# maoqingyu1996/Boosting-Neural-Video-Representation-via-Online-Structural-Reparameteration

Hardware: AMD Instinct MI355X
Metric: training frames/sec, Bunny 720p ERB (higher is better)
Workload: dtype f16; 1 GPU; configs[1]: Bunny-shaped 132x3x720x1280 synthetic video, branch_type=ERB, fc_hw_dim 9_16_26, strides 5 2 2 2 2, stem 512_1, lower_width 96, Fusion6, Adam(0.5,0.999), b=1; one independent video per GPU; precision=fp16, hip_graph=False, launch_mode=stream, finite=True

## Files before the change

boosting-neural-video-representation-via-online-structural-reparameteration_amd/_lib.py:

```python
import ctypes
import os
from ctypes import POINTER, c_char_p, c_double, c_float, c_int, c_int32, c_int64, c_size_t, c_void_p

HERE = os.path.dirname(os.path.abspath(__file__))
ORN_MAX_LAYERS = 8
LOSS_TYPES = {'L2': 0, 'L1': 1, 'Fusion6': 2}


class OrnError(RuntimeError):
    pass


def lib_path() -> str:
    return os.environ.get('ORN_LIB_PATH') or os.path.join(HERE, 'liborn.so')


class LayerDesc(ctypes.Structure):
    _fields_ = [('C', c_int32), ('O', c_int32), ('s', c_int32), ('H', c_int32), ('W', c_int32),
                ('w3x3', c_int64), ('b3x3', c_int64), ('w3x1', c_int64), ('b3x1', c_int64),
                ('w1x3', c_int64), ('b1x3', c_int64), ('w1', c_int64), ('w2', c_int64), ('w3', c_int64)]


class EngineDesc(ctypes.Structure):
    _fields_ = [('n_layers', c_int32), ('erb', c_int32), ('embed_len', c_int32), ('stem_dim', c_int32),
# ... 54 lines not shown
    'orn_engine_train_steps': (c_int, [P, P, P, P, P, P, c_int32, c_int32, P]),
    'orn_engine_profile_step': (c_int, [P, P, P, P, P, P, c_int32, P, P]),
    'orn_engine_set_grad_mask': (c_int, [P, P]),
    'orn_engine_set_target_stats': (c_int, [P, P]),
    'orn_engine_fused_kernel': (c_int, [P, c_int, POINTER(c_void_p), POINTER(c_void_p)]),
    'orn_engine_scale_state': (c_int, [P, P]),
    'orn_engine_set_grad_scale': (c_int, [P, c_float, c_float]),
}
EXPORTS = tuple(_SIGS.keys())
_DEBUG_SIGS = {'orn_debug_set': (None, [c_int]), 'orn_debug_set_stamps': (None, [c_void_p]),
               'orn_debug_conv_fwd_bf16': (c_int, [P, P, P] + [c_int] * 5 + [P, P, c_int, P]),
               'orn_debug_conv_fwd_f16': (c_int, [P, P, P] + [c_int] * 5 + [P, P, c_int, P]),
               'orn_debug_conv_dgrad_bf16': (c_int, [P, P] + [c_int] * 4 + [P, P, c_int, P, c_int, P]),
               'orn_debug_conv_dgrad_f16': (c_int, [P, P] + [c_int] * 4 + [P, P, c_int, P, c_int, P]),
               'orn_debug_merge_h16_bwd': (c_int, [c_int, P, P, P, P, P]),
               'orn_debug_decode_out_ws_bytes': (c_size_t, []),
               'orn_debug_decode_out_f32': (c_int, [P, c_int, c_int, P, P, P, P, P, c_size_t, P])}

_lib = None


def lib():
    global _lib
    if _lib is None:
        path = lib_path()
        if not os.path.exists(path):
            raise OrnError(f'{path} is missing: build it with `python -c "import __graft_entry__ as g; g.build()"` '
                           '(hipcc --offload-arch=gfx950).  There is no CPU fallback.')
        L = ctypes.CDLL(path)
        for name, (res, args) in _SIGS.items():
# ... 37 lines not shown
```

boosting-neural-video-representation-via-online-structural-reparameteration_amd/csrc/orn_engine.hip:

```cpp
#include "orn_internal.h"
#include <new>
#include <cstdlib>
#include <cassert>

struct LayerBuf {
    float *T, *wf, *bf;
    float *w2t;
    float *dT, *dw1p;
    float *wd32;
    void *mh16;
    float *dw2t;
    float *z, *a;
    float *da;
    uint16_t *xpad;
    uint16_t *zb;
    uint16_t *dypad;
    uint16_t *wb, *wd;
    float *biasp;
    float *wslab;
};

struct orn_engine {
    orn_engine_desc d;
    float *params, *grads, *m, *v;
    const float *gmask;
    const float *tstats;
    float *ws;
    float *pre1, *h1, *pre2, *h2, *dh2;
    float *img, *dimg, *stats;
// ... 13 lines not shown
        int layer[ORN_MAX_LAYERS];
        void *tables;
        int tiles[4];
        void *mh_tables, *mh_host;
    } mset[3];
    int ff;
    float *dxn;
    size_t stem_ws;
    bool stage0;
    hipGraph_t graph, graph_u;
    hipGraphExec_t graph_exec, graph_exec_u;
    const void *g_frames, *g_embeds, *g_sched, *g_cursor, *g_stats;
    int g_slots;
    hipStream_t g_stream;
    hipStream_t side;
    hipEvent_t ev_fork, ev_adam, ev_wgrad, ev_join, ev_below;
    OrnStepCur *cur_side;
    OrnScaleState *sc_side;
    size_t side_lo;
    bool pipe_ok;
    bool side_below;
    bool fork_behind_dgrad;
    int last_smax;
    bool side_busy;
    bool prof;
    hipEvent_t prof_ev[4 * ORN_MAX_LAYERS + 4];
};

#define ORN_GRAPH_UNROLL 4
static_assert(ORN_SCALE_SLOTS >= ORN_GRAPH_UNROLL, "one scale-state entry per step of the unrolled graph");

static inline size_t al(size_t floats) { return orn_align(floats * 4) / 4; }

static hipEvent_t orn_engine::*const SIDE_EVENTS[] = {&orn_engine::ev_fork, &orn_engine::ev_adam, &orn_engine::ev_wgrad, &orn_engine::ev_join,
                                                      &orn_engine::ev_below};

static constexpr int ORN_LAST_SMAX = 24;

static void drop_graphs(orn_engine *e)
{
    if (e->graph_exec) { (void)hipGraphExecDestroy(e->graph_exec); e->graph_exec = nullptr; }
    if (e->graph) { (void)hipGraphDestroy(e->graph); e->graph = nullptr; }
    if (e->graph_exec_u) { (void)hipGraphExecDestroy(e->graph_exec_u); e->graph_exec_u = nullptr; }
    if (e->graph_u) { (void)hipGraphDestroy(e->graph_u); e->graph_u = nullptr; }
}

extern "C" size_t orn_conv3x3_ps_silu_bwd_ws_bytes(int B, int C, int O, int H, int W);
extern "C" size_t orn_erb_merge_bwd_ws_bytes(int C, int O);
extern "C" size_t orn_head_bwd_ws_bytes(int B, int C, int H, int W);
extern "C" size_t orn_loss_ws_bytes(int B, int Ch, int H, int W);
// ... 100 lines not shown
    if (s3 > scratch) scratch = s3;
    float *scr = take(scratch);
    const orn_layer_desc &ll = d->layer[d->n_layers - 1];
    float *head_ws = (ff < d->n_layers) ? take(orn_half_ops_bf16()->head_bwd_ws_floats(Cn))
                   : (ll.s == 2 ? take((size_t)(orn_head_bwd_fused_f32_blocks(ll.H, ll.W) + 1) * (3 * Cn + 3)) : nullptr);
    float *cur = take((sizeof(OrnStepCur) * ORN_GRAPH_UNROLL + 3) / 4 + 16);
    float *scs = take(sizeof(OrnScaleState) * ORN_SCALE_SLOTS / 4);
    float *mtab[3], *mhtab[3];
    for (int k = 0; k < 3; ++k) {
        mtab[k] = d->erb ? take(orn_merge_group_bytes() / 4) : nullptr;
        mhtab[k] = (d->erb && d->precision != 0) ? take(orn_merge_h16_table_bytes() / 4) : nullptr;
    }
    float *cur_side = take((sizeof(OrnStepCur) + 3) / 4 + 16);
    float *sc_side = take(sizeof(OrnScaleState) / 4 + 16);
    float *dec_ws = take(ORN_DECODE_WS_FLOATS);
    if (e) {
        e->pre1 = pre1; e->h1 = h1; e->pre2 = pre2; e->h2 = h2; e->dh2 = dh2;
        e->img = img; e->dimg = dimg; e->stats = stats; e->loss_ws = loss_ws; e->scratch = scr; e->head_ws = head_ws;
        e->cur = (OrnStepCur *)cur;
        e->sc = (OrnScaleState *)scs;
        for (int i = 0; i < d->n_layers; ++i) e->L[i] = L[i];
        e->Hout = H; e->Wout = W; e->Cn_last = Cn;
        e->ff = ff; e->dxn = dxn;
        e->stem_ws = al(orn_stem_bwd_ws_floats(1, d->stem_dim, Nout));
        const orn_layer_desc &l0 = d->layer[0];
        e->stage0 = d->precision != 0 && ff == 1 && d->n_layers > 1 && orn_stage0_supported(l0.C, l0.O, l0.H, l0.W, l0.s);
        for (int k = 0; k < 3; ++k) { e->mset[k].tables = mtab[k]; e->mset[k].mh_tables = mhtab[k]; }
        e->cur_side = (OrnStepCur *)cur_side;
        e->sc_side = (OrnScaleState *)sc_side;
        e->dec_ws = dec_ws;
// ... 20 lines not shown
        return ORN_E_WS;
    }
    ORN_TRY(orn_loss_init());
    orn_engine *e = new (std::nothrow) orn_engine();
    ORN_REQUIRE(e, "engine_create: out of host memory");
    e->d = *d;
    e->params = params; e->grads = grads; e->m = adam_m; e->v = adam_v;
    e->gmask = nullptr;
    e->tstats = nullptr;
    e->ws = (float *)ws;
    e->graph = nullptr; e->graph_exec = nullptr; e->graph_u = nullptr; e->graph_exec_u = nullptr;
    e->prof = false;
    for (int k = 0; k < 3; ++k) { e->mset[k].n = 0; e->mset[k].mh_host = nullptr; }
    e->side = nullptr;
    for (auto ev : SIDE_EVENTS) e->*ev = nullptr;
    e->pipe_ok = false; e->side_busy = false; e->side_lo = 0;
    for (int i = 0; i < 4 * ORN_MAX_LAYERS + 4; ++i) e->prof_ev[i] = nullptr;
    e->ops = (d->precision == 2) ? orn_half_ops_f16() : orn_half_ops_bf16();
    e->gs = (d->precision == 2) ? 1048576.0f : 1.0f;
    layout(d, e);
    {
        hipError_t rc = hipMemset(ws, 0, need);
        if (rc == hipSuccess) rc = hipDeviceSynchronize();
        if (rc != hipSuccess) { orn_set_error("engine_create: hipMemset failed: %s", hipGetErrorString(rc)); delete e; return (int)rc; }
        OrnScaleState s0[ORN_SCALE_SLOTS] = {};
        for (int r = 0; r < ORN_SCALE_SLOTS; ++r) { s0[r].gs = e->gs; s0[r].inv_gs = 1.0f / e->gs; s0[r].gs_max = e->gs; }
        rc = hipMemcpy(e->sc, s0, sizeof(s0), hipMemcpyHostToDevice);
        if (rc == hipSuccess) rc = hipMemcpy(e->sc_side, s0, sizeof(OrnScaleState), hipMemcpyHostToDevice);
        if (rc != hipSuccess) { orn_set_error("engine_create: scale state upload failed: %s", hipGetErrorString(rc)); delete e; return (int)rc; }
    }
    {
// ... 29 lines not shown
            e->L[i].wf = params + d->layer[i].w3x3;
            e->L[i].bf = params + d->layer[i].b3x3;
        }
    else {
        auto fill = [&](int i, OrnMergeLayer &m, bool half_in_S) {
            const orn_layer_desc &l = d->layer[i];
            m.C = l.C; m.O = l.O;
            m.w3x3 = params + l.w3x3; m.w3x1 = params + l.w3x1; m.w1x3 = params + l.w1x3;
            m.w1 = params + l.w1; m.w2 = params + l.w2; m.w3 = params + l.w3;
            m.T = e->L[i].T; m.wf = e->L[i].wf; m.w2t = e->L[i].w2t;
            m.b3x3 = params + l.b3x3; m.b1x3 = params + l.b1x3; m.b3x1 = params + l.b3x1; m.bf = e->L[i].bf;
            m.g = grads ? grads + l.w3x3 : nullptr;
            m.dT = e->L[i].dT; m.dw1p = e->L[i].dw1p;
            m.dw2 = grads ? grads + l.w2 : nullptr; m.dw3 = grads ? grads + l.w3 : nullptr;
            m.dw2t = e->L[i].dw2t;
            m.half_kind = 0; m.s2 = l.s * l.s; m.Cp = ORN_FAST_C; m.wb = m.wd = nullptr; m.biasp = nullptr;
            if (i >= e->ff && half_in_S) {
                m.half_kind = d->precision; m.wb = e->L[i].wb; m.wd = e->L[i].wd; m.biasp = e->L[i].biasp;
            }
        };
        const int nl = d->n_layers;
        for (int k = 0; k < (e->pipe_ok ? 3 : 1); ++k) {
            orn_engine::MergeSet &ms = e->mset[k];
            const int i0 = k == 2 ? nl - 1 : 0, i1 = k == 1 ? nl - 1 : nl;
            ms.n = 0;
            void *bufs[ORN_MAX_LAYERS];
            for (int i = i0; i < i1; ++i) {
                fill(i, ms.ml[ms.n], k == 2 || !e->stage0);
                bufs[ms.n] = e->L[i].mh16;
                ms.layer[ms.n++] = i;
// ... 122 lines not shown

static bool f32_head_on_z(const orn_engine *e)
{
    const orn_engine_desc &d = e->d;
    return e->ff >= d.n_layers && e->head_ws && d.layer[d.n_layers - 1].s == 2;
}

static int slab_cap(const orn_engine *e, int i) { return i == e->d.n_layers - 1 ? e->last_smax : 0; }

static OrnPrepLayer prep_layer(const orn_engine *e, int i)
{
    const orn_layer_desc &l = e->d.layer[i];
    return OrnPrepLayer{e->L[i].wf, e->L[i].bf, l.O, l.C, l.s, e->L[i].wb, e->L[i].wd, e->L[i].biasp, ORN_FAST_C};
}

static OrnWgradJob wgrad_job(const orn_engine *e, int i)
{
    const orn_layer_desc &l = e->d.layer[i];
    return OrnWgradJob{e->L[i].xpad, e->L[i].dypad, l.H, l.W, l.C, l.O, l.s, e->L[i].wslab, slab_cap(e, i)};
}

static OrnWgradReduce wgrad_reduce(const orn_engine *e, int i, OrnScaleState *sc)
{
    const orn_layer_desc &l = e->d.layer[i];
    return OrnWgradReduce{e->L[i].wslab, l.H, l.W, l.C, l.O, l.s, 1.0f / e->gs, e->grads + l.w3x3, e->grads + l.b3x3, sc, slab_cap(e, i)};
}

enum { MERGE_NONE = -1 };
static int forward(orn_engine *e, const float *embeds, const int *row_idx, bool keep_z, hipStream_t st, int set = 0, bool head = true)
{
    const bool merge = set != MERGE_NONE;
    const orn_engine_desc &d = e->d;
    const int Nout = d.fc_h * d.fc_w * d.fc_dim;
    float *P = e->params;
    const OrnLinearJob lin1 = {embeds, row_idx, (size_t)d.embed_len, P + d.stem_w0, P + d.stem_b0, 1, d.embed_len, d.stem_dim, e->pre1, e->h1};
    const OrnLinearJob lin2 = {e->h1, nullptr, 0, P + d.stem_w1, P + d.stem_b1, 1, d.stem_dim, Nout, e->pre2, e->h2};
    const float *x = e->h2;
    const int nl = d.n_layers, ff = e->ff;
    const void *pack_t = nullptr;
    int pack_t_blocks = 0;
// ... 28 lines not shown
                ORN_TRY(orn_launch_stage0_fwd(x, b.wf, b.bf, l.C, l.O, l.H, l.W, l.s, keep_z ? b.z : nullptr, e->L[1].xpad, ORN_FAST_C,
                                              d.precision, st, np, pl, pack_t, pack_t_blocks));
            }
            else
            {
                const bool z_only = keep_z && i == nl - 1 && f32_head_on_z(e);
                ORN_TRY(orn_launch_conv3x3_f32(x, b.wf, b.bf, 1, l.C, l.O, l.H, l.W, l.s, 1, keep_z ? b.z : nullptr, z_only ? nullptr : b.a, st, nullptr));
            }
            if (e->prof) (void)hipEventRecord(e->prof_ev[2 * i + 1], st);
            x = b.a;
        } else {
            if (i == ff && !e->stage0) ORN_TRY(e->ops->to_nhwc(x, l.C, ORN_FAST_C, l.H, l.W, b.xpad, st));
            if (e->prof) (void)hipEventRecord(e->prof_ev[2 * i], st);
            const bool last = (i + 1 == nl);
            if (e->side_busy && i + 3 == nl && e->side_below) ORN_HIP(hipStreamWaitEvent(st, e->ev_below, 0));
            if (e->side_busy && i + 2 == nl) ORN_HIP(hipStreamWaitEvent(st, e->ev_wgrad, 0));
            if (e->side_busy && last) { ORN_HIP(hipStreamWaitEvent(st, e->ev_join, 0)); e->side_busy = false; }
            ORN_TRY(e->ops->conv_fwd(b.xpad, b.wb, b.biasp, l.H, l.W, ORN_FAST_C, l.O, l.s, b.zb, last ? nullptr : e->L[i + 1].xpad, st, l.C));
            if (e->prof) (void)hipEventRecord(e->prof_ev[2 * i + 1], st);
        }
    }
    if (ff < nl) {
        if (head)
            ORN_TRY(e->ops->head_fwd(e->L[nl - 1].zb, P + d.head_w, P + d.head_b, e->Cn_last, (size_t)e->Hout * e->Wout, d.sigmoid, e->img, st));
    } else
    {
        const bool z_only = keep_z && f32_head_on_z(e);
        ORN_TRY(orn_launch_head_fwd(z_only ? e->L[nl - 1].z : x, P + d.head_w, P + d.head_b, 1, e->Cn_last, (size_t)e->Hout * e->Wout, d.sigmoid, e->img,
                                    st, z_only));
    }
    return 0;
}

// ... 93 lines not shown
    const orn_engine_desc &d = e->d;
    const int nl = d.n_layers;
    float *G = e->grads;
    hipStream_t sd = e->side;
    OrnScaleState *sc = e->sc_side;
    ORN_HIP(hipEventRecord(e->ev_fork, st));
    ORN_HIP(hipStreamWaitEvent(sd, e->ev_fork, 0));
    if (e->side_below) {
        const OrnWgradJob wb = wgrad_job(e, nl - 2);
        ORN_TRY(e->ops->wgrad_batch(1, &wb, sd, nullptr, nullptr, 1));
        ORN_HIP(hipEventRecord(e->ev_below, sd));
    }
    const OrnWgradJob wj = wgrad_job(e, nl - 1);
    const OrnHeadFinish hf = {e->head_ws, e->ops->head_bwd_blocks(e->Hout, e->Wout), e->Cn_last, 1.0f / e->gs, G + d.head_w, G + d.head_b, sc};
    ORN_TRY(e->ops->wgrad_batch(1, &wj, sd, &hf, nullptr, 1));
    ORN_HIP(hipEventRecord(e->ev_wgrad, sd));
    const OrnWgradReduce wr = wgrad_reduce(e, nl - 1, sc);
    ORN_TRY(e->ops->wgrad_reduce_all(1, &wr, sd, nullptr));
    if (d.erb) {
        const orn_engine::MergeSet &ms = e->mset[2];
        ORN_TRY(orn_launch_merge_h16_bwd(ms.mh_tables, ms.mh_host, sd, sc));
        const OrnMergeMisc mm = merge_misc(e, nl - 1);
        ORN_TRY(orn_launch_merge_bwd_tail_all(1, &mm, sd));
    }
    return 0;
}

static int side_branch_update(orn_engine *e, bool more)
{
    const orn_engine_desc &d = e->d;
    const int nl = d.n_layers;
// ... 157 lines not shown
    ORN_REQUIRE(e->grads && e->m && e->v, "engine_train_step: engine was created without grads / Adam arenas");
    return train_step(e, frames, embeds, sched, cursor, stats_out, n_slots, (hipStream_t)stream);
}

extern "C" int orn_engine_train_steps(orn_engine *e, const float *frames, const float *embeds, const orn_step_sched *sched,
                                      int32_t *cursor, float *stats_out, int32_t n_slots, int32_t n_steps, void *stream)
{
    ORN_REQUIRE(e && frames && embeds && sched && cursor && n_steps >= 0, "engine_train_steps: bad arguments");
    ORN_REQUIRE(e->grads && e->m && e->v, "engine_train_steps: engine was created without grads / Adam arenas");
    hipStream_t st = (hipStream_t)stream;
    int rc = 0;
    StepOpts o;
    o.pipe = e->pipe_ok;
    for (int k = 0; k < n_steps && rc == 0; ++k) {
        o.more = k + 1 < n_steps;
        rc = train_step(e, frames, embeds, sched, cursor, stats_out, n_slots, st, o);
    }
    if (e->side_busy) {
        const hipError_t hrc = hipStreamWaitEvent(st, e->ev_join, 0);
        e->side_busy = false;
        if (hrc != hipSuccess && rc == 0) { orn_set_error("engine_train_steps: join: %s", hipGetErrorString(hrc)); rc = (int)hrc; }
    }
    return rc;
}

extern "C" int orn_engine_profile_step(orn_engine *e, const float *frames, const float *embeds, const orn_step_sched *sched,
                                       int32_t *cursor, float *stats_out, int32_t n_slots, float *ms_out, void *stream)
{
    ORN_REQUIRE(e && frames && embeds && sched && cursor && ms_out, "engine_profile_step: null pointer");
    ORN_REQUIRE(e->grads && e->m && e->v, "engine_profile_step: engine was created without grads / Adam arenas");
    hipStream_t st = (hipStream_t)stream;
    const int nl = e->d.n_layers;
// ... 79 lines not shown
```

boosting-neural-video-representation-via-online-structural-reparameteration_amd/csrc/orn_internal.h:

```cpp
#pragma once
#include "orn_common.h"

int orn_launch_linear_silu(const float *x, const int *row_idx, size_t row_stride, const float *w, const float *b,
                           int B, int K, int N, float *pre, float *y, hipStream_t st);
int orn_launch_stem_bwd(const float *embed, const int *row_idx, size_t row_stride, const float *w1, const float *pre1,
                        const float *h1, const float *pre2, const float *dh2, int B, int E, int Hd, int Nout,
                        float *dw0, float *db0, float *dw1, float *db1, float *ws, hipStream_t st, int dh2_nslab = 1,
                        OrnStemW0Job *defer_w0 = nullptr,
                        OrnStemL2Job *defer_l2 = nullptr);
size_t orn_stem_bwd_ws_floats(int B, int Hd, int Nout);
int orn_launch_head_fwd(const float *a, const float *w, const float *b, int B, int C, size_t HW, int sigmoid,
                        float *out, hipStream_t st, bool z_input = false);
int orn_launch_head_bwd(const float *a, const float *w, const float *out, const float *dout, int B, int C, size_t HW,
                        int sigmoid, float *da, float *dw, float *db, float *ws, hipStream_t st);
int orn_launch_adam(float *p, const float *g, float *m, float *v, size_t n, double lr, int step, const OrnStepCur *sp,
                    double beta1, double beta2, double eps, float inv_gscale, hipStream_t st, const float *gmask = nullptr,
                    OrnScaleState *sc = nullptr,
                    OrnScaleState *sc_master = nullptr,
                    OrnScaleState *mirror = nullptr,
                    bool count_skip = true,
                    OrnScaleState *late = nullptr);

bool orn_stage0_supported(int C, int O, int H, int W, int s);
int orn_stage0_slabs(int O, int s);
// ... 9 lines not shown
                         const float *w1x3, const float *b1x3, const float *w1, const float *w2, const float *w3,
                         int C, int O, float *T, float *wf, float *bf, hipStream_t st);
int orn_launch_merge_bwd(const float *g, const float *dbf, const float *w1, const float *w2, const float *w3,
                         const float *T, int C, int O, float *d3x3, float *db3x3, float *d3x1, float *db3x1,
                         float *d1x3, float *db1x3, float *dw1, float *dw2, float *dw3, float *ws, hipStream_t st);

struct OrnMergeLayer {
    int C, O;
    const float *w3x3, *w3x1, *w1x3, *w1, *w2, *w3;
    const float *b3x3, *b1x3, *b3x1; float *bf;
    float *T, *wf;
    float *w2t;
    const float *g;
    float *dT, *dw1p, *dw2, *dw3;
    float *dw2t;
    int half_kind, s2, Cp;
    void *wb, *wd;
    float *biasp;
};
size_t orn_merge_group_bytes();
int orn_launch_w2_transpose(int n_layers, const OrnMergeLayer *L, hipStream_t st, const void *pack = nullptr, int par_blocks = 0);
int orn_merge_groups_build(void *dev_tables, int n_layers, const OrnMergeLayer *L, bool fp32_bwd, int tiles[4]);
int orn_launch_merge_group(const void *dev_tables, int which, int tiles, hipStream_t st);
int orn_launch_merge_group_linear(const void *dev_tables, int which, int tiles, const OrnLinearJob &job, hipStream_t st,
                                  const void *pack = nullptr, int pack_blocks = 0);

size_t orn_merge_h16_layer_halfs(int C, int O);
size_t orn_merge_h16_table_bytes();
size_t orn_merge_h16_host_bytes();
int orn_merge_h16_build(void *dev_tables, void *host, int n_layers, const OrnMergeLayer *L, void *const *bufs, OrnScaleState *sc);
int orn_launch_merge_h16_bwd(const void *dev_tables, const void *host, hipStream_t st, OrnScaleState *sc = nullptr);
const void *orn_merge_h16_pack(const void *host, int *par_blocks, int *t_blocks);
int orn_launch_merge_h16_pack_jobs(const void *host, int which, hipStream_t st);

struct OrnMergeMisc {
    int C, O;
    const float *g, *dbf, *dw1p;
    float *d3x1, *db3x1, *d1x3, *db1x3, *dw1;
    const float *dw2t; float *dw2;
};
int orn_launch_merge_bwd_tail_all(int n, const OrnMergeMisc *L, hipStream_t st);

int orn_launch_conv3x3_f32(const float *x, const float *w, const float *bias, int B, int C, int O, int H, int W,
                           int s, int epi, float *z, float *out, hipStream_t st, float *split_ws);
struct OrnHeadBwdFuse { const float *w, *out, *dout; int sigmoid; float *dw, *db, *hws; };
// ... 4 lines not shown
int orn_head_bwd_fused_f32_blocks(int H, int W);
int orn_launch_head_bwd_fused_f32(const float *z, const float *w, const float *out, const float *dout, int Cn, int H, int W,
                                  int sigmoid, float *dy, float *dbp, float *dw, float *db, float *hws, hipStream_t st);

int orn_loss_init();
int orn_launch_loss(const float *pred, const float *target, const int *frame_idx, size_t frame_stride, int B, int Ch,
                    int H, int W, int loss_type, float loss_scale, float *stats, float *dpred, float *ws,
                    hipStream_t st, const OrnStepCur *cur = nullptr, float *ring = nullptr, OrnScaleState *sc = nullptr,
                    const float *tstats = nullptr,
                    OrnLossFinalJob *defer = nullptr);
int orn_msssim_frames_chunk(int n, int Ch, int H, int W, size_t ws_bytes);
int orn_launch_msssim_frames(const float *pred, const float *targets, const int32_t *rows, int F, int Ch, int H, int W, float *out,
                             float *ws, hipStream_t st);

struct OrnPrepLayer { const float *wf, *bf; int O, C, s; void *wb, *wd; float *biasp; int Cp; };
struct OrnWgradReduce { const float *slabs; int H, W, C, O, s; float gscale; float *dwf, *dbf; OrnScaleState *sc; int smax; };
struct OrnHeadFinish { const float *partial; int blocks, C; float gscale; float *dw, *db; OrnScaleState *sc; };
struct OrnWgradJob { const void *xpad, *dypad; int H, W, C, O, s; float *slabs; int smax; };
#define ORN_DECODE_MAX_BLOCKS 8192
#define ORN_DECODE_WS_FLOATS (2 * ORN_DECODE_MAX_BLOCKS + 64)
struct OrnDecodeOut { const float *targets; const int32_t *row; uint8_t *rgb8; float *img, *stats; float *ws; };
int orn_launch_decode_out_f32(const float *src, size_t HW, const OrnDecodeOut &o, hipStream_t st);
struct OrnHalfOps {
    int (*conv_fwd)(const void *xpad, const void *wb, const float *bias_p, int H, int W, int Cin, int O, int s, void *z, void *apad,
                    hipStream_t st, int c_real);
    int (*conv_dgrad)(const void *dypad, const void *wd, int H, int W, int O, int C, const void *zprev, void *dyprev, int sp,
                      float *dx_f32, hipStream_t st, int c_real);
    size_t (*wgrad_ws_floats)(int H, int W, int O);
    int (*wgrad_batch)(int n, const OrnWgradJob *J, hipStream_t st, const OrnHeadFinish *hf, const OrnStemL2Job *l2, int side);
    int (*wgrad_reduce_all)(int n, const OrnWgradReduce *L, hipStream_t st, const OrnStemW0Job *w0);
    int (*prep_all)(int n, const OrnPrepLayer *L, hipStream_t st);
// ... 14 lines not shown
```

boosting-neural-video-representation-via-online-structural-reparameteration_amd/csrc/orn_merge_h16.hip:

```cpp
#include "orn_internal.h"
#include "orn_merge_pack.h"
#include <new>

typedef __attribute__((ext_vector_type(8))) _Float16 mh16x8;
typedef __attribute__((ext_vector_type(16))) float mf32x16;


struct MhSizes { size_t gh, gt, th, w3t, w1h, w2p, dtt, dtc; };
static MhSizes mh_sizes(int C, int O)
{
    const int E = 9 * C, K2 = 2 * C;
    MhSizes s;
    s.gh = (size_t)r32(O) * r16(E);
    s.gt = (size_t)r32(E) * r16(O);
    s.th = (size_t)r32(O) * r16(E);
    s.w3t = (size_t)r32(O) * r16(O);
    s.w1h = (size_t)r32(K2) * r16(C);
    s.w2p = (size_t)9 * r32(K2) * r16(O);
    s.dtt = (size_t)9 * r32(O) * r16(C);
    s.dtc = (size_t)9 * r32(C) * r16(O);
    return s;
}

size_t orn_merge_h16_layer_halfs(int C, int O)
// ... 150 lines not shown
    H->pack.sc = sc;
    H->pack.grad_start[0] = 0;
    H->pack.par_start[0] = 0;
    H->pack.tt_start[0] = 0;
    for (int i = 0; i < n_layers; ++i) {
        const OrnMergeLayer &l = L[i];
        const int C = l.C, O = l.O, E = 9 * C, K2 = 2 * C;
        const MhSizes s = mh_sizes(C, O);
        mh16 *base = (mh16 *)bufs[i];
        auto take = [&](size_t n) { mh16 *p = base; base += (n + 127) / 128 * 128; return p; };
        mh16 *gh = take(s.gh), *gt = take(s.gt), *th = take(s.th), *w3t = take(s.w3t), *w1h = take(s.w1h), *w2p = take(s.w2p);
        mh16 *dtt = take(s.dtt), *dtc = take(s.dtc);
        H->pack.l[i] = MhPackLayer{C, O, l.g, l.T, l.w1, l.w2, l.w3, gh, gt, th, w3t, w1h, w2p};
        const int jobs[MH_JOBS] = {orn_cdiv((long)O * E, 256 * MH_CPT), orn_cdiv((long)O * E, 256 * MH_CPT), orn_cdiv((long)K2 * C, 256 * MH_CPT),
                                   orn_cdiv(O, 64) * orn_cdiv(E, 64), orn_cdiv(O, 64) * orn_cdiv(O, 64), orn_cdiv(O, 64) * orn_cdiv(K2 * 9, 64)};
        H->pack.grad_start[2 * i + 1] = H->pack.grad_start[2 * i] + jobs[0];
        H->pack.grad_start[2 * i + 2] = H->pack.grad_start[2 * i + 1] + jobs[3];
        const int pj[3] = {jobs[2], jobs[4], jobs[5]};
        for (int j = 0; j < 3; ++j) H->pack.par_start[3 * i + j + 1] = H->pack.par_start[3 * i + j] + pj[j];
        H->pack.tt_start[i + 1] = H->pack.tt_start[i] + jobs[1];
        MhProb p;
        p = MhProb{};
        p.A = gh; p.lda = r16(E); p.B = th; p.ldb = r16(E); p.M = O; p.N = O; p.K = r16(E); p.nbatch = 1;
        p.mode = 0; p.C = l.dw3; p.scm = O; p.scn = 1; p.so = 1.0f / MH_GS;
        mh_add(G[0], p);
        p = MhProb{};
        p.A = w3t; p.lda = r16(O); p.B = gt; p.ldb = r16(O); p.M = O; p.N = E; p.K = r16(O); p.nbatch = 1;
        p.mode = 1; p.dtt = dtt; p.dtc = dtc; p.Cch = C; p.ldt = r16(C); p.ldc = r16(O);
        p.st_t = (long)r32(O) * r16(C); p.st_c = (long)r32(C) * r16(O);
        mh_add(G[0], p);
        p = MhProb{};
        p.A = dtt; p.lda = r16(C); p.ba = (long)r32(O) * r16(C); p.B = w1h; p.ldb = r16(C); p.bb = 0;
// ... 5 lines not shown
        p.M = K2; p.N = C; p.K = r16(O); p.nbatch = 9;
        p.mode = 0; p.C = l.dw1p; p.scm = C; p.scn = 1; p.bc = (long)K2 * C; p.so = 1.0f / MH_GS;
        mh_add(G[1], p);
    }
    H->pack_blocks_grad = H->pack.grad_start[2 * n_layers];
    H->pack_blocks_par = H->pack.par_start[3 * n_layers];
    H->pack_blocks_t = H->pack.tt_start[n_layers];
    H->tiles[0] = G[0].tile_start[G[0].n];
    H->tiles[1] = G[1].tile_start[G[1].n];
    hipError_t e = hipMemcpy(dev_tables, G, 2 * sizeof(MhGroup), hipMemcpyHostToDevice);
    delete[] G;
    if (e != hipSuccess) { orn_set_error("merge h16: hipMemcpy failed: %s", hipGetErrorString(e)); return (int)e; }
    return 0;
}

const void *orn_merge_h16_pack(const void *host, int *par_blocks, int *t_blocks)
{
    const OrnMergeH16 *H = (const OrnMergeH16 *)host;
    *par_blocks = H->pack_blocks_par;
    *t_blocks = H->pack_blocks_t;
    return &H->pack;
}

int orn_launch_merge_h16_pack_jobs(const void *host, int which, hipStream_t st)
{
    const OrnMergeH16 *H = (const OrnMergeH16 *)host;
    const int blocks = which == MH_TAB_PAR ? H->pack_blocks_par : H->pack_blocks_t;
    if (blocks <= 0) return 0;
    hipLaunchKernelGGL(k_merge_pack, dim3(blocks), dim3(256), 0, st, H->pack, which);
    ORN_LAUNCH_CHECK("merge_pack(jobs)");
    return 0;
}

int orn_launch_merge_h16_bwd(const void *dev_tables, const void *host, hipStream_t st, OrnScaleState *sc)
{
    const OrnMergeH16 *H = (const OrnMergeH16 *)host;
    MhPackAll pack = H->pack;
    if (sc) pack.sc = sc;
    hipLaunchKernelGGL(k_merge_pack, dim3(H->pack_blocks_grad), dim3(256), 0, st, pack, (int)MH_TAB_GRAD);
    ORN_LAUNCH_CHECK("merge_pack");
    const MhGroup *g = (const MhGroup *)dev_tables;
    hipLaunchKernelGGL(k_mgemm_h16, dim3(H->tiles[0]), dim3(256), 0, st, g, H->tiles[0], pack.sc);
    ORN_LAUNCH_CHECK("mgemm_h16(dW3,dT)");
    hipLaunchKernelGGL(k_mgemm_h16, dim3(H->tiles[1]), dim3(256), 0, st, g + 1, H->tiles[1], (OrnScaleState *)nullptr);
    ORN_LAUNCH_CHECK("mgemm_h16(dW2,dW1)");
    return 0;
}

extern "C" int orn_debug_merge_h16_bwd(int n, const int *co, const float *const *in, float *const *out, int *flag, void *stream)
{
    ORN_REQUIRE(n >= 1 && n <= ORN_MAX_LAYERS && co && in && out && flag, "debug_merge_h16_bwd: bad arguments");
    for (int i = 0; i < n; ++i) ORN_REQUIRE(co[2 * i] >= 1 && co[2 * i + 1] >= 1, "debug_merge_h16_bwd: layer %d: C, O >= 1", i);
    hipStream_t st = (hipStream_t)stream;
    const size_t a0 = 256, a1 = a0 + orn_align(orn_merge_h16_table_bytes());
    size_t off[ORN_MAX_LAYERS][3], tot = a1;
// ... 29 lines not shown
    hipError_t e = hipSuccess;
    if (rc == 0 && (e = hipMemset(ws, 0, tot)) == hipSuccess) e = hipMemcpy(sc, &s0, sizeof(s0), hipMemcpyHostToDevice);
    if (rc == 0 && e != hipSuccess) { orn_set_error("debug_merge_h16_bwd: %s", hipGetErrorString(e)); rc = (int)e; }
    if (rc == 0) rc = orn_merge_h16_build(ws + a0, host, n, L, bufs, sc);
    if (rc == 0) rc = orn_launch_merge_h16_pack_jobs(host, MH_TAB_PAR, st);
    if (rc == 0) rc = orn_launch_merge_h16_pack_jobs(host, MH_TAB_T, st);
    if (rc == 0) rc = orn_launch_merge_h16_bwd(ws + a0, host, st, sc);
    if (rc == 0) rc = orn_launch_merge_bwd_tail_all(n, M, st);
    if (rc == 0 && (e = hipStreamSynchronize(st)) == hipSuccess) e = hipMemcpy(&s0, sc, sizeof(s0), hipMemcpyDeviceToHost);
    if (rc == 0 && e != hipSuccess) { orn_set_error("debug_merge_h16_bwd: %s", hipGetErrorString(e)); rc = (int)e; }
    if (rc == 0) *flag = s0.flag;
    free(host);
    (void)hipFree(ws);
    return rc;
}
```

boosting-neural-video-representation-via-online-structural-reparameteration_amd/csrc/orn_wgrad_bf16.hip:

```cpp
#include "orn_h16.h"

namespace HNS {

#include "orn_wgrad_body.h"
static int g_wgrad_dbg = 0;
void set_debug_wgrad(int flags) { g_wgrad_dbg = flags; }

__global__ void __launch_bounds__(256, 2) k_wgrad_nhwc_bf16(WgradBP p) { wgrad_body(p, blockIdx.x); }

__device__ __forceinline__ void head_finish_body(const float *__restrict__ partial, int blocks, int C, float gscale, float *__restrict__ dw,
                                                 float *__restrict__ db, int col, float *sred , OrnScaleState *sc = nullptr)
{
    if (sc) gscale = sc->inv_gs;
    const int n = 3 * C + 3, t = threadIdx.x;
    float acc = 0.f;
    for (int r = t; r < blocks; r += 256) acc += partial[(size_t)r * n + col];
    sred[t] = acc;
    __syncthreads();
    for (int w = 128; w > 0; w >>= 1) {
        if (t < w) sred[t] += sred[t + w];
        __syncthreads();
    }
    if (t == 0) {
        const float v = sred[0] * gscale;
// ... 28 lines not shown
    }
    if ((int)blockIdx.x >= a.start[a.n]) {
        extern __shared__ __attribute__((aligned(16))) unsigned char smem_hf[];
        head_finish_body(a.hf.partial, a.hf.blocks, a.hf.C, a.hf.gscale, a.hf.dw, a.hf.db, (int)blockIdx.x - a.start[a.n],
                         reinterpret_cast<float *>(smem_hf), a.hf.sc);
        return;
    }
    int k = 0;
    while (k + 1 < a.n && (int)blockIdx.x >= a.start[k + 1]) ++k;
    k = __builtin_amdgcn_readfirstlane(k);
    wgrad_body(a.p[k], (int)blockIdx.x - a.start[k]);
}

__device__ __forceinline__ void wgrad_reduce_body(const float *__restrict__ slabs, const float *__restrict__ bias_slabs, int S, int O, int Cn,
                                                  int s2, int Cr, float gscale, float *__restrict__ dwf, float *__restrict__ dbf,
                                                  OrnScaleState *sc = nullptr)
{
    if (sc) gscale = sc->inv_gs;
    const size_t n = (size_t)9 * O * 96;
    const size_t idx = (size_t)blockIdx.x * blockDim.x + threadIdx.x;
    if (idx < (size_t)O && dbf) {
        float b = 0.f;
        for (int s = 0; s < S; ++s) b += bias_slabs[(size_t)s * O + idx];
        const int ij = (int)idx / Cn, nn = (int)idx - ij * Cn;
        dbf[nn * s2 + ij] = b * gscale;
        orn_flag_nonfinite(sc, b * gscale);
    }
    if (idx >= n) return;
    const int c = (int)(idx % 96);
    if (c >= Cr) return;
    float a8[8] = {0.f, 0.f, 0.f, 0.f, 0.f, 0.f, 0.f, 0.f};
    int s = 0;
    for (; s + 8 <= S; s += 8) {
#pragma unroll
        for (int k = 0; k < 8; ++k) a8[k] += slabs[(size_t)(s + k) * n + idx];
    }
    for (; s < S; ++s) a8[0] += slabs[(size_t)s * n + idx];
    const float acc = ((a8[0] + a8[1]) + (a8[2] + a8[3])) + ((a8[4] + a8[5]) + (a8[6] + a8[7]));
    const size_t r = idx / 96;
    const int op = (int)(r % O), tap = (int)(r / O);
    const int ij = op / Cn, nn = op - ij * Cn;
    const int o = nn * s2 + ij;
    dwf[((size_t)o * Cr + c) * 9 + tap] = acc * gscale;
    orn_flag_nonfinite(sc, acc * gscale);
}

__global__ void k_wgrad_bf16_reduce(const float *__restrict__ slabs, const float *__restrict__ bias_slabs, int S, int O, int Cn,
                                    int s2, int Cr, float gscale, float *__restrict__ dwf, float *__restrict__ dbf)
{
    wgrad_reduce_body(slabs, bias_slabs, S, O, Cn, s2, Cr, gscale, dwf, dbf);
}

struct WgradReduceAll {
    struct { const float *slabs, *bias_slabs; int S, O, Cn, s2, Cr; float gscale; float *dwf, *dbf; OrnScaleState *sc; } l[ORN_MAX_LAYERS];
    int n; OrnStemW0Job w0;
};
__global__ void k_wgrad_bf16_reduce_all(WgradReduceAll a)
{
    if ((int)blockIdx.y == a.n) {
        __shared__ float sh_w0[4];
        if (2 * (int)blockIdx.x >= a.w0.N) return;
        const int half = threadIdx.x >> 7;
        orn_stem_w0_row(a.w0, (int)blockIdx.x * 2 + half, threadIdx.x & 127, sh_w0 + 2 * half);
        return;
    }
    const auto &l = a.l[blockIdx.y];
    if ((size_t)blockIdx.x * blockDim.x >= (size_t)9 * l.O * 96) return;
    wgrad_reduce_body(l.slabs, l.bias_slabs, l.S, l.O, l.Cn, l.s2, l.Cr, l.gscale, l.dwf, l.dbf, l.sc);
}

int orn_wgrad_bf16_split(int H, int W, int O, int smax = 0)
{
    const int n_ktiles = orn_cdiv(H, WB_TH) * orn_cdiv(W, WB_TW);
    const int per = 3 * orn_cdiv(O, WB_BO);
    int S = (512 / per) / 8 * 8;
    if (S > 40) S = 40;
    if (n_ktiles < 2000 && S > 24 && smax < 8) S = 24;
    const int by_work = (n_ktiles / 8) / 8 * 8;
    if (S > by_work) S = by_work;
    if (smax >= 8 && S > smax) S = smax / 8 * 8;
    if (S < 8) S = 8;
    return S;
}
// ... 59 lines not shown
    if (!dwf) return 0;
    const size_t n = (size_t)9 * O * 96;
    hipLaunchKernelGGL(k_wgrad_bf16_reduce, dim3(orn_cdiv((long)n, 256)), dim3(256), 0, st, slabs, p.bias_slabs, p.S, O,
                       O / (s * s), s * s, C, gscale, dwf, dbf);
    ORN_LAUNCH_CHECK("wgrad_bf16_reduce");
    return 0;
}

int orn_launch_wgrad_reduce_all(int n, const OrnWgradReduce *L, hipStream_t st, const OrnStemW0Job *w0)
{
    if (n == 0 && !w0) return 0;
    ORN_REQUIRE(n <= ORN_MAX_LAYERS, "wgrad_reduce_all: %d layers", n);
    WgradReduceAll a;
    size_t mx = 0;
    for (int i = 0; i < n; ++i) {
        const int S = orn_wgrad_bf16_split(L[i].H, L[i].W, L[i].O, L[i].smax), s2 = L[i].s * L[i].s;
        a.l[i].slabs = L[i].slabs; a.l[i].bias_slabs = L[i].slabs + (size_t)S * 9 * L[i].O * 96;
        a.l[i].S = S; a.l[i].O = L[i].O; a.l[i].Cn = L[i].O / s2; a.l[i].s2 = s2; a.l[i].Cr = L[i].C; a.l[i].gscale = L[i].gscale;
        a.l[i].dwf = L[i].dwf; a.l[i].dbf = L[i].dbf; a.l[i].sc = L[i].sc;
        const size_t w = (size_t)9 * L[i].O * 96;
        if (w > mx) mx = w;
    }
    a.n = n;
    a.w0 = OrnStemW0Job{};
    if (w0) { a.w0 = *w0; const size_t need = (size_t)orn_cdiv(w0->N, 2) * 256; if (need > mx) mx = need; }
    hipLaunchKernelGGL(k_wgrad_bf16_reduce_all, dim3(orn_cdiv((long)mx, 256), n + (w0 ? 1 : 0)), dim3(256), 0, st, a);
    ORN_LAUNCH_CHECK("wgrad_bf16_reduce_all");
    return 0;
}

}
```

include/orn_debug.h:

```cpp
#ifndef ORN_DEBUG_H_
#define ORN_DEBUG_H_
#include "orn.h"
#ifdef __cplusplus
extern "C" {
#endif
ORN_API void orn_debug_set(int flags);
ORN_API int orn_debug_conv_fwd_bf16(const void *xpad, const void *wb, const float *bias_p, int H, int W, int Cin, int O, int s,
                                    void *z, void *apad, int c_real, void *stream);
ORN_API int orn_debug_conv_fwd_f16(const void *xpad, const void *wb, const float *bias_p, int H, int W, int Cin, int O, int s,
                                   void *z, void *apad, int c_real, void *stream);
ORN_API int orn_debug_conv_dgrad_bf16(const void *dypad, const void *wd, int H, int W, int O, int C, const void *zprev,
                                      void *dyprev, int sp, float *dx_f32, int c_real, void *stream);
ORN_API int orn_debug_conv_dgrad_f16(const void *dypad, const void *wd, int H, int W, int O, int C, const void *zprev,
                                     void *dyprev, int sp, float *dx_f32, int c_real, void *stream);
ORN_API int orn_debug_merge_h16_bwd(int n, const int *co, const float *const *in, float *const *out, int *flag, void *stream);
ORN_API size_t orn_debug_decode_out_ws_bytes(void);
ORN_API int orn_debug_decode_out_f32(const float *img, int H, int W, const float *target, uint8_t *rgb8, float *img_out,
                                     float *stats, void *ws, size_t ws_bytes, void *stream);
#ifdef ORN_CONV_STAMP
ORN_API void orn_debug_set_stamps(void *buf);
#endif
#ifdef __cplusplus
}
#endif
#endif
```

Before: 988.2 frames/s.

## Double-buffer last-layer input and fuse f16 gradient packing into wgrad reduce

Adds a second padded input buffer for the last layer and alternates between the two buffers on pipelined steps. The next step's forward conv can then write its input while the side-stream wgrad of the previous step is still reading the old one, which lets the ev_wgrad wait be removed. The wgrad reduce also writes the half-precision Gh/GT gradient copies directly, so the separate merge-pack gradient jobs are skipped for fast layers, and the slab summation loop is unrolled by 24. The cost is extra memory, more complex buffer selection, and a debug entry point for checking the fused pack.

Result: no change. 982.6 frames/s (-0.6%).

```diff
diff --git a/boosting-neural-video-representation-via-online-structural-reparameteration_amd/_lib.py b/boosting-neural-video-representation-via-online-structural-reparameteration_amd/_lib.py
--- a/boosting-neural-video-representation-via-online-structural-reparameteration_amd/_lib.py
+++ b/boosting-neural-video-representation-via-online-structural-reparameteration_amd/_lib.py
@@ -92,6 +92,7 @@
                'orn_debug_conv_dgrad_bf16': (c_int, [P, P] + [c_int] * 4 + [P, P, c_int, P, c_int, P]),
                'orn_debug_conv_dgrad_f16': (c_int, [P, P] + [c_int] * 4 + [P, P, c_int, P, c_int, P]),
                'orn_debug_merge_h16_bwd': (c_int, [c_int, P, P, P, P, P]),
+               'orn_debug_wgrad_reduce_pack': (c_int, [P] + [c_int] * 5 + [P] * 6),
                'orn_debug_decode_out_ws_bytes': (c_size_t, []),
                'orn_debug_decode_out_f32': (c_int, [P, c_int, c_int, P, P, P, P, P, c_size_t, P])}
 
diff --git a/boosting-neural-video-representation-via-online-structural-reparameteration_amd/csrc/orn_engine.hip b/boosting-neural-video-representation-via-online-structural-reparameteration_amd/csrc/orn_engine.hip
--- a/boosting-neural-video-representation-via-online-structural-reparameteration_amd/csrc/orn_engine.hip
+++ b/boosting-neural-video-representation-via-online-structural-reparameteration_amd/csrc/orn_engine.hip
@@ -13,6 +13,7 @@
     float *z, *a;
     float *da;
     uint16_t *xpad;
+    uint16_t *xpad1;
     uint16_t *zb;
     uint16_t *dypad;
     uint16_t *wb, *wd;
@@ -56,7 +57,8 @@
     int g_slots;
     hipStream_t g_stream;
     hipStream_t side;
-    hipEvent_t ev_fork, ev_adam, ev_wgrad, ev_join, ev_below;
+    hipEvent_t ev_fork, ev_adam, ev_join, ev_below;
+    int xsel;
     OrnStepCur *cur_side;
     OrnScaleState *sc_side;
     size_t side_lo;
@@ -74,8 +76,7 @@
 
 static inline size_t al(size_t floats) { return orn_align(floats * 4) / 4; }
 
-static hipEvent_t orn_engine::*const SIDE_EVENTS[] = {&orn_engine::ev_fork, &orn_engine::ev_adam, &orn_engine::ev_wgrad, &orn_engine::ev_join,
-                                                      &orn_engine::ev_below};
+static hipEvent_t orn_engine::*const SIDE_EVENTS[] = {&orn_engine::ev_fork, &orn_engine::ev_adam, &orn_engine::ev_join, &orn_engine::ev_below};
 
 static constexpr int ORN_LAST_SMAX = 24;
 
@@ -206,6 +207,11 @@
     float *cur_side = take((sizeof(OrnStepCur) + 3) / 4 + 16);
     float *sc_side = take(sizeof(OrnScaleState) / 4 + 16);
     float *dec_ws = take(ORN_DECODE_WS_FLOATS);
+    if (d->precision != 0 && ff < d->n_layers - 1) {
+        const orn_layer_desc &l = d->layer[d->n_layers - 1];
+        L[d->n_layers - 1].xpad1 = (uint16_t *)take(((size_t)(l.H + 2) * (l.W + 2) * ORN_FAST_C + 1) / 2);
+        take((size_t)(l.W + 2) * ORN_FAST_C / 2);
+    }
     if (e) {
         e->pre1 = pre1; e->h1 = h1; e->pre2 = pre2; e->h2 = h2; e->dh2 = dh2;
         e->img = img; e->dimg = dimg; e->stats = stats; e->loss_ws = loss_ws; e->scratch = scr; e->head_ws = head_ws;
@@ -256,7 +262,7 @@
     for (int k = 0; k < 3; ++k) { e->mset[k].n = 0; e->mset[k].mh_host = nullptr; }
     e->side = nullptr;
     for (auto ev : SIDE_EVENTS) e->*ev = nullptr;
-    e->pipe_ok = false; e->side_busy = false; e->side_lo = 0;
+    e->pipe_ok = false; e->side_busy = false; e->side_lo = 0; e->xsel = 0;
     for (int i = 0; i < 4 * ORN_MAX_LAYERS + 4; ++i) e->prof_ev[i] = nullptr;
     e->ops = (d->precision == 2) ? orn_half_ops_f16() : orn_half_ops_bf16();
     e->gs = (d->precision == 2) ? 1048576.0f : 1.0f;
@@ -316,6 +322,7 @@
             m.dT = e->L[i].dT; m.dw1p = e->L[i].dw1p;
             m.dw2 = grads ? grads + l.w2 : nullptr; m.dw3 = grads ? grads + l.w3 : nullptr;
             m.dw2t = e->L[i].dw2t;
+            m.g_packed = i >= e->ff;
             m.half_kind = 0; m.s2 = l.s * l.s; m.Cp = ORN_FAST_C; m.wb = m.wd = nullptr; m.biasp = nullptr;
             if (i >= e->ff && half_in_S) {
                 m.half_kind = d->precision; m.wb = e->L[i].wb; m.wd = e->L[i].wd; m.biasp = e->L[i].biasp;
@@ -468,16 +475,23 @@
     return OrnPrepLayer{e->L[i].wf, e->L[i].bf, l.O, l.C, l.s, e->L[i].wb, e->L[i].wd, e->L[i].biasp, ORN_FAST_C};
 }
 
+static uint16_t *xpad_of(const orn_engine *e, int i)
+{
+    return (i == e->d.n_layers - 1 && e->xsel) ? e->L[i].xpad1 : e->L[i].xpad;
+}
+
 static OrnWgradJob wgrad_job(const orn_engine *e, int i)
 {
     const orn_layer_desc &l = e->d.layer[i];
-    return OrnWgradJob{e->L[i].xpad, e->L[i].dypad, l.H, l.W, l.C, l.O, l.s, e->L[i].wslab, slab_cap(e, i)};
+    return OrnWgradJob{xpad_of(e, i), e->L[i].dypad, l.H, l.W, l.C, l.O, l.s, e->L[i].wslab, slab_cap(e, i)};
 }
 
 static OrnWgradReduce wgrad_reduce(const orn_engine *e, int i, OrnScaleState *sc)
 {
     const orn_layer_desc &l = e->d.layer[i];
-    return OrnWgradReduce{e->L[i].wslab, l.H, l.W, l.C, l.O, l.s, 1.0f / e->gs, e->grads + l.w3x3, e->grads + l.b3x3, sc, slab_cap(e, i)};
+    OrnWgradReduce r = {e->L[i].wslab, l.H, l.W, l.C, l.O, l.s, 1.0f / e->gs, e->grads + l.w3x3, e->grads + l.b3x3, sc, slab_cap(e, i), nullptr, nullptr, 0};
+    if (e->d.erb && e->L[i].mh16) orn_merge_h16_grad_copies(e->L[i].mh16, l.C, l.O, &r.gh, &r.gt);
+    return r;
 }
 
 enum { MERGE_NONE = -1 };
@@ -536,9 +550,8 @@
             if (e->prof) (void)hipEventRecord(e->prof_ev[2 * i], st);
             const bool last = (i + 1 == nl);
             if (e->side_busy && i + 3 == nl && e->side_below) ORN_HIP(hipStreamWaitEvent(st, e->ev_below, 0));
-            if (e->side_busy && i + 2 == nl) ORN_HIP(hipStreamWaitEvent(st, e->ev_wgrad, 0));
             if (e->side_busy && last) { ORN_HIP(hipStreamWaitEvent(st, e->ev_join, 0)); e->side_busy = false; }
-            ORN_TRY(e->ops->conv_fwd(b.xpad, b.wb, b.biasp, l.H, l.W, ORN_FAST_C, l.O, l.s, b.zb, last ? nullptr : e->L[i + 1].xpad, st, l.C));
+            ORN_TRY(e->ops->conv_fwd(xpad_of(e, i), b.wb, b.biasp, l.H, l.W, ORN_FAST_C, l.O, l.s, b.zb, last ? nullptr : xpad_of(e, i + 1), st, l.C));
             if (e->prof) (void)hipEventRecord(e->prof_ev[2 * i + 1], st);
         }
     }
@@ -662,7 +675,6 @@
     const OrnWgradJob wj = wgrad_job(e, nl - 1);
     const OrnHeadFinish hf = {e->head_ws, e->ops->head_bwd_blocks(e->Hout, e->Wout), e->Cn_last, 1.0f / e->gs, G + d.head_w, G + d.head_b, sc};
     ORN_TRY(e->ops->wgrad_batch(1, &wj, sd, &hf, nullptr, 1));
-    ORN_HIP(hipEventRecord(e->ev_wgrad, sd));
     const OrnWgradReduce wr = wgrad_reduce(e, nl - 1, sc);
     ORN_TRY(e->ops->wgrad_reduce_all(1, &wr, sd, nullptr));
     if (d.erb) {
@@ -850,8 +862,10 @@
     o.pipe = e->pipe_ok;
     for (int k = 0; k < n_steps && rc == 0; ++k) {
         o.more = k + 1 < n_steps;
+        e->xsel = o.pipe ? (k & 1) : 0;
         rc = train_step(e, frames, embeds, sched, cursor, stats_out, n_slots, st, o);
     }
+    e->xsel = 0;
     if (e->side_busy) {
         const hipError_t hrc = hipStreamWaitEvent(st, e->ev_join, 0);
         e->side_busy = false;
diff --git a/boosting-neural-video-representation-via-online-structural-reparameteration_amd/csrc/orn_internal.h b/boosting-neural-video-representation-via-online-structural-reparameteration_amd/csrc/orn_internal.h
--- a/boosting-neural-video-representation-via-online-structural-reparameteration_amd/csrc/orn_internal.h
+++ b/boosting-neural-video-representation-via-online-structural-reparameteration_amd/csrc/orn_internal.h
@@ -47,6 +47,7 @@
     const float *g;
     float *dT, *dw1p, *dw2, *dw3;
     float *dw2t;
+    bool g_packed;
     int half_kind, s2, Cp;
     void *wb, *wd;
     float *biasp;
@@ -62,6 +63,7 @@
 size_t orn_merge_h16_table_bytes();
 size_t orn_merge_h16_host_bytes();
 int orn_merge_h16_build(void *dev_tables, void *host, int n_layers, const OrnMergeLayer *L, void *const *bufs, OrnScaleState *sc);
+void orn_merge_h16_grad_copies(void *buf, int C, int O, void **gh, void **gt);
 int orn_launch_merge_h16_bwd(const void *dev_tables, const void *host, hipStream_t st, OrnScaleState *sc = nullptr);
 const void *orn_merge_h16_pack(const void *host, int *par_blocks, int *t_blocks);
 int orn_launch_merge_h16_pack_jobs(const void *host, int which, hipStream_t st);
@@ -96,7 +98,7 @@
                              float *ws, hipStream_t st);
 
 struct OrnPrepLayer { const float *wf, *bf; int O, C, s; void *wb, *wd; float *biasp; int Cp; };
-struct OrnWgradReduce { const float *slabs; int H, W, C, O, s; float gscale; float *dwf, *dbf; OrnScaleState *sc; int smax; };
+struct OrnWgradReduce { const float *slabs; int H, W, C, O, s; float gscale; float *dwf, *dbf; OrnScaleState *sc; int smax; void *gh, *gt; int S; };
 struct OrnHeadFinish { const float *partial; int blocks, C; float gscale; float *dw, *db; OrnScaleState *sc; };
 struct OrnWgradJob { const void *xpad, *dypad; int H, W, C, O, s; float *slabs; int smax; };
 #define ORN_DECODE_MAX_BLOCKS 8192
diff --git a/boosting-neural-video-representation-via-online-structural-reparameteration_amd/csrc/orn_merge_h16.hip b/boosting-neural-video-representation-via-online-structural-reparameteration_amd/csrc/orn_merge_h16.hip
--- a/boosting-neural-video-representation-via-online-structural-reparameteration_amd/csrc/orn_merge_h16.hip
+++ b/boosting-neural-video-representation-via-online-structural-reparameteration_amd/csrc/orn_merge_h16.hip
@@ -188,8 +188,8 @@
         H->pack.l[i] = MhPackLayer{C, O, l.g, l.T, l.w1, l.w2, l.w3, gh, gt, th, w3t, w1h, w2p};
         const int jobs[MH_JOBS] = {orn_cdiv((long)O * E, 256 * MH_CPT), orn_cdiv((long)O * E, 256 * MH_CPT), orn_cdiv((long)K2 * C, 256 * MH_CPT),
                                    orn_cdiv(O, 64) * orn_cdiv(E, 64), orn_cdiv(O, 64) * orn_cdiv(O, 64), orn_cdiv(O, 64) * orn_cdiv(K2 * 9, 64)};
-        H->pack.grad_start[2 * i + 1] = H->pack.grad_start[2 * i] + jobs[0];
-        H->pack.grad_start[2 * i + 2] = H->pack.grad_start[2 * i + 1] + jobs[3];
+        H->pack.grad_start[2 * i + 1] = H->pack.grad_start[2 * i] + (l.g_packed ? 0 : jobs[0]);
+        H->pack.grad_start[2 * i + 2] = H->pack.grad_start[2 * i + 1] + (l.g_packed ? 0 : jobs[3]);
         const int pj[3] = {jobs[2], jobs[4], jobs[5]};
         for (int j = 0; j < 3; ++j) H->pack.par_start[3 * i + j + 1] = H->pack.par_start[3 * i + j] + pj[j];
         H->pack.tt_start[i + 1] = H->pack.tt_start[i] + jobs[1];
@@ -225,6 +225,13 @@
     return 0;
 }
 
+void orn_merge_h16_grad_copies(void *buf, int C, int O, void **gh, void **gt)
+{
+    const MhSizes s = mh_sizes(C, O);
+    *gh = buf;
+    *gt = (mh16 *)buf + (s.gh + 127) / 128 * 128;
+}
+
 const void *orn_merge_h16_pack(const void *host, int *par_blocks, int *t_blocks)
 {
     const OrnMergeH16 *H = (const OrnMergeH16 *)host;
@@ -248,8 +255,10 @@
     const OrnMergeH16 *H = (const OrnMergeH16 *)host;
     MhPackAll pack = H->pack;
     if (sc) pack.sc = sc;
-    hipLaunchKernelGGL(k_merge_pack, dim3(H->pack_blocks_grad), dim3(256), 0, st, pack, (int)MH_TAB_GRAD);
-    ORN_LAUNCH_CHECK("merge_pack");
+    if (H->pack_blocks_grad > 0) {
+        hipLaunchKernelGGL(k_merge_pack, dim3(H->pack_blocks_grad), dim3(256), 0, st, pack, (int)MH_TAB_GRAD);
+        ORN_LAUNCH_CHECK("merge_pack");
+    }
     const MhGroup *g = (const MhGroup *)dev_tables;
     hipLaunchKernelGGL(k_mgemm_h16, dim3(H->tiles[0]), dim3(256), 0, st, g, H->tiles[0], pack.sc);
     ORN_LAUNCH_CHECK("mgemm_h16(dW3,dT)");
@@ -309,3 +318,39 @@
     (void)hipFree(ws);
     return rc;
 }
+
+extern "C" int orn_debug_wgrad_reduce_pack(const float *slabs, int S, int O, int s, int Cr, int fused, float *dwf, float *dbf,
+                                           void *gh, void *gt, int *flag, void *stream)
+{
+    ORN_REQUIRE(slabs && dwf && dbf && gh && gt && flag, "debug_wgrad_reduce_pack: null pointer");
+    ORN_REQUIRE(S >= 1 && s >= 1 && O >= 1 && O % (s * s) == 0 && Cr >= 1 && Cr <= 96, "debug_wgrad_reduce_pack: bad S=%d O=%d s=%d Cr=%d", S, O, s, Cr);
+    hipStream_t st = (hipStream_t)stream;
+    OrnScaleState *sc = nullptr;
+    ORN_HIP(hipMalloc(&sc, sizeof(OrnScaleState)));
+    OrnScaleState s0 = {};
+    s0.gs = s0.inv_gs = s0.gs_max = 1.0f;
+    hipError_t e = hipMemcpy(sc, &s0, sizeof(s0), hipMemcpyHostToDevice);
+    int rc = 0;
+    if (e == hipSuccess) {
+        OrnWgradReduce wr = {};
+        wr.slabs = slabs; wr.C = Cr; wr.O = O; wr.s = s; wr.gscale = 1.0f; wr.dwf = dwf; wr.dbf = dbf; wr.sc = sc; wr.S = S;
+        if (fused) { wr.gh = gh; wr.gt = gt; }
+        rc = orn_half_ops_f16()->wgrad_reduce_all(1, &wr, st, nullptr);
+        if (rc == 0 && !fused) {
+            MhPackAll pack = {};
+            const int E = 9 * Cr;
+            pack.n = 1;
+            pack.sc = sc;
+            pack.l[0] = MhPackLayer{Cr, O, dwf, nullptr, nullptr, nullptr, nullptr, (mh16 *)gh, (mh16 *)gt, nullptr, nullptr, nullptr, nullptr};
+            pack.grad_start[1] = orn_cdiv((long)O * E, 256 * MH_CPT);
+            pack.grad_start[2] = pack.grad_start[1] + orn_cdiv(O, 64) * orn_cdiv(E, 64);
+            hipLaunchKernelGGL(k_merge_pack, dim3(pack.grad_start[2]), dim3(256), 0, st, pack, (int)MH_TAB_GRAD);
+            e = hipGetLastError();
+        }
+        if (rc == 0 && e == hipSuccess && (e = hipStreamSynchronize(st)) == hipSuccess) e = hipMemcpy(&s0, sc, sizeof(s0), hipMemcpyDeviceToHost);
+    }
+    (void)hipFree(sc);
+    if (rc == 0 && e != hipSuccess) { orn_set_error("debug_wgrad_reduce_pack: %s", hipGetErrorString(e)); rc = (int)e; }
+    if (rc == 0) *flag = s0.flag;
+    return rc;
+}
diff --git a/boosting-neural-video-representation-via-online-structural-reparameteration_amd/csrc/orn_wgrad_bf16.hip b/boosting-neural-video-representation-via-online-structural-reparameteration_amd/csrc/orn_wgrad_bf16.hip
--- a/boosting-neural-video-representation-via-online-structural-reparameteration_amd/csrc/orn_wgrad_bf16.hip
+++ b/boosting-neural-video-representation-via-online-structural-reparameteration_amd/csrc/orn_wgrad_bf16.hip
@@ -1,4 +1,5 @@
 #include "orn_h16.h"
+#include "orn_merge_pack.h"
 
 namespace HNS {
 
@@ -66,7 +67,7 @@
 
 __device__ __forceinline__ void wgrad_reduce_body(const float *__restrict__ slabs, const float *__restrict__ bias_slabs, int S, int O, int Cn,
                                                   int s2, int Cr, float gscale, float *__restrict__ dwf, float *__restrict__ dbf,
-                                                  OrnScaleState *sc = nullptr)
+                                                  OrnScaleState *sc = nullptr, mh16 *__restrict__ gh = nullptr, mh16 *__restrict__ gt = nullptr)
 {
     if (sc) gscale = sc->inv_gs;
     const size_t n = (size_t)9 * O * 96;
@@ -83,6 +84,15 @@
     if (c >= Cr) return;
     float a8[8] = {0.f, 0.f, 0.f, 0.f, 0.f, 0.f, 0.f, 0.f};
     int s = 0;
+    for (; s + 24 <= S; s += 24) {
+        float v[24];
+#pragma unroll
+        for (int k = 0; k < 24; ++k) v[k] = slabs[(size_t)(s + k) * n + idx];
+#pragma unroll
+        for (int j = 0; j < 3; ++j)
+#pragma unroll
+            for (int k = 0; k < 8; ++k) a8[k] += v[8 * j + k];
+    }
     for (; s + 8 <= S; s += 8) {
 #pragma unroll
         for (int k = 0; k < 8; ++k) a8[k] += slabs[(size_t)(s + k) * n + idx];
@@ -93,8 +103,16 @@
     const int op = (int)(r % O), tap = (int)(r / O);
     const int ij = op / Cn, nn = op - ij * Cn;
     const int o = nn * s2 + ij;
-    dwf[((size_t)o * Cr + c) * 9 + tap] = acc * gscale;
-    orn_flag_nonfinite(sc, acc * gscale);
+    const float g = acc * gscale;
+    dwf[((size_t)o * Cr + c) * 9 + tap] = g;
+    orn_flag_nonfinite(sc, g);
+    if (gh) {
+        const mh16 hv = (mh16)(g * MH_GS);
+        const int e = c * 9 + tap;
+        gh[(size_t)o * r16(9 * Cr) + e] = hv;
+        gt[(size_t)e * r16(O) + o] = hv;
+        if (!(fabsf((float)hv) <= 3.0e38f)) orn_flag_nonfinite(sc, __builtin_nanf(""));
+    }
 }
 
 __global__ void k_wgrad_bf16_reduce(const float *__restrict__ slabs, const float *__restrict__ bias_slabs, int S, int O, int Cn,
@@ -104,7 +122,7 @@
 }
 
 struct WgradReduceAll {
-    struct { const float *slabs, *bias_slabs; int S, O, Cn, s2, Cr; float gscale; float *dwf, *dbf; OrnScaleState *sc; } l[ORN_MAX_LAYERS];
+    struct { const float *slabs, *bias_slabs; int S, O, Cn, s2, Cr; float gscale; float *dwf, *dbf; OrnScaleState *sc; mh16 *gh, *gt; } l[ORN_MAX_LAYERS];
     int n; OrnStemW0Job w0;
 };
 __global__ void k_wgrad_bf16_reduce_all(WgradReduceAll a)
@@ -118,7 +136,7 @@
     }
     const auto &l = a.l[blockIdx.y];
     if ((size_t)blockIdx.x * blockDim.x >= (size_t)9 * l.O * 96) return;
-    wgrad_reduce_body(l.slabs, l.bias_slabs, l.S, l.O, l.Cn, l.s2, l.Cr, l.gscale, l.dwf, l.dbf, l.sc);
+    wgrad_reduce_body(l.slabs, l.bias_slabs, l.S, l.O, l.Cn, l.s2, l.Cr, l.gscale, l.dwf, l.dbf, l.sc, l.gh, l.gt);
 }
 
 int orn_wgrad_bf16_split(int H, int W, int O, int smax = 0)
@@ -208,10 +226,12 @@
     WgradReduceAll a;
     size_t mx = 0;
     for (int i = 0; i < n; ++i) {
-        const int S = orn_wgrad_bf16_split(L[i].H, L[i].W, L[i].O, L[i].smax), s2 = L[i].s * L[i].s;
+        ORN_REQUIRE(!L[i].gh == !L[i].gt && (!L[i].gh || L[i].sc), "wgrad_reduce_all: layer %d: Gh and GT come together, with a scale state", i);
+        const int S = L[i].S > 0 ? L[i].S : orn_wgrad_bf16_split(L[i].H, L[i].W, L[i].O, L[i].smax), s2 = L[i].s * L[i].s;
         a.l[i].slabs = L[i].slabs; a.l[i].bias_slabs = L[i].slabs + (size_t)S * 9 * L[i].O * 96;
         a.l[i].S = S; a.l[i].O = L[i].O; a.l[i].Cn = L[i].O / s2; a.l[i].s2 = s2; a.l[i].Cr = L[i].C; a.l[i].gscale = L[i].gscale;
         a.l[i].dwf = L[i].dwf; a.l[i].dbf = L[i].dbf; a.l[i].sc = L[i].sc;
+        a.l[i].gh = (mh16 *)L[i].gh; a.l[i].gt = (mh16 *)L[i].gt;
         const size_t w = (size_t)9 * L[i].O * 96;
         if (w > mx) mx = w;
     }
diff --git a/include/orn_debug.h b/include/orn_debug.h
--- a/include/orn_debug.h
+++ b/include/orn_debug.h
@@ -14,6 +14,8 @@
 ORN_API int orn_debug_conv_dgrad_f16(const void *dypad, const void *wd, int H, int W, int O, int C, const void *zprev,
                                      void *dyprev, int sp, float *dx_f32, int c_real, void *stream);
 ORN_API int orn_debug_merge_h16_bwd(int n, const int *co, const float *const *in, float *const *out, int *flag, void *stream);
+ORN_API int orn_debug_wgrad_reduce_pack(const float *slabs, int S, int O, int s, int Cr, int fused, float *dwf, float *dbf,
+                                        void *gh, void *gt, int *flag, void *stream);
 ORN_API size_t orn_debug_decode_out_ws_bytes(void);
 ORN_API int orn_debug_decode_out_f32(const float *img, int H, int W, const float *target, uint8_t *rgb8, float *img_out,
                                      float *stats, void *ws, size_t ws_bytes, void *stream);
```
